# flanglet/kanzi

Hardware: AMD Instinct MI355X
Metric: encode+decode MB/s, 4 MiB-block synthetic stream, BWT+RANK+ZRLT & ANS0 (level-5 core chain), bit-exact .knz (higher is better)
Workload: dtype u8; 1 GPU; configs[2]: BWT+RANK+ZRLT & ANS0, 2048 x 4194304 B blocks per GPU per step (64 distinct synthetic blocks per GPU, SURVEY 8d generator standing in for silesia.tar, tiled), blocks round-robin over ranks; block_size=4194304, parallelism=blocks%1, round_trip_ok=True

## Files before the change

kanzi_amd/csrc/kz_ans.hip:

```cpp
#include "kz_device.h"
#include "kz_internal.h"
#include "kz_chunk.h"

typedef uint16_t u16;

#define ANS_TOP (1u << 15)
#define ANS_LR 12


struct BitW { u8* p; u32 pos; };
__device__ __forceinline__ void bw_put(BitW& w, u32 v, int count) {
  while (count > 0) {
    const int bitoff = w.pos & 7, room = 8 - bitoff;
    const int take = count < room ? count : room;
    const u32 bits = (v >> (count - take)) & ((1u << take) - 1u);
    w.p[w.pos >> 3] |= (u8)(bits << (room - take));
    w.pos += take; count -= take;
  }
}

typedef u16 __attribute__((aligned(1))) ans_u16_unaligned;
typedef u64 __attribute__((aligned(1))) ans_u64_unaligned;

__global__ __launch_bounds__(64) void k_ans_enc_chunk(const u8* __restrict__ src, int64_t stride,
                                                       const int32_t* __restrict__ d_len, AnsEnc E) {
  const int b = blockIdx.y, ck = blockIdx.x;
  const int count = d_len[b];
  const int lane = kz_lane();
  const int64_t ci = (int64_t)b * E.C + ck;
  const u8* blk = src + (int64_t)b * stride;
  u8* hdr = E.hdr + ci * ANS_HDR_BYTES;
  u8* scr = E.scr + ci * ANS_SCRATCH;
  if (count <= 32) {
    if (ck != 0) return;
    if (lane < count) scr[lane] = blk[lane];
    if (lane == 0) { E.hdrBits[ci] = 0; E.tailOff[ci] = 0; E.tailBits[ci] = 8u * (u32)count; }
    return;
  }
  const int start = ck * ANS_CHUNK;
  if (start >= count) return;
  const int end = min(count, start + ANS_CHUNK);
  const int len = end - start;

  __shared__ u32 hist[256];
  __shared__ u16 nfreq[256];
  __shared__ u8 alpha[256];
  __shared__ uint4 symTab[256];
  const u8* data = blk + start;
  __shared__ u32 hbuf[ANS_HDR_BYTES / 4];

  for (int i = lane; i < 256; i += 64) hist[i] = 0;
  for (int i = lane; i < ANS_HDR_BYTES / 4; i += 64) hbuf[i] = 0;
  __syncthreads();
  for (int i = lane * 4; i < len; i += 256) {
    u32 w = 0; int nb = min(4, len - i);
    if (nb == 4 && ((start + i) & 3) == 0) w = *(const u32*)(blk + start + i);
    else for (int k = 0; k < nb; k++) w |= (u32)blk[start + i + k] << (8 * k);
    for (int k = 0; k < 4; k++) {
      const bool valid = k < nb;
      const u32 c = (w >> (8 * k)) & 0xFF;
      const uint64_t peers = kz_match8(c, valid);
      if (valid && (peers & kz_lanemask_lt()) == 0) atomicAdd(&hist[c], (u32)__popcll(peers));
    }
  }
  __syncthreads();

  const u32 total = (u32)len, scale = 1u << ANS_LR;
  u32 f[4]; bool present[4];
  u32 alphabetSize = 0;
  u32 apos[4];
#pragma unroll
  for (int q = 0; q < 4; q++) {
    f[q] = hist[q * 64 + lane];
// ... 58 lines not shown
          if (adjustments == 0) break;
        }
#pragma unroll
        for (int q = 0; q < 4; q++) if (q == mq && lane == ml) { int v = (int)f[q] - delta; f[q] = (u32)(v > 1 ? v : 1); }
      }
      if (adjMax != 0) {
#pragma unroll
        for (int q = 0; q < 4; q++) if (q == mq && lane == ml) f[q] = (u32)((int)f[q] + adjMax);
      }
    }
  }
  u32 cum = 0;
#pragma unroll
  for (int q = 0; q < 4; q++) {
    const u32 fv = present[q] ? f[q] : 0;
    const u32 inc = kz_wave_incl_sum(fv);
    const u32 cumFreq = cum + inc - fv;
    cum += __shfl(inc, 63, 64);
    const int s = q * 64 + lane;
    nfreq[s] = (u16)fv;
    if (present[q]) {
      u32 freq = fv;
      if (freq >= scale) freq = scale - 1;
      const u32 xmaxv = ((ANS_TOP >> ANS_LR) << 16) * freq;
      const u32 cmplv = scale - freq;
      if (freq < 2) symTab[s] = make_uint4(xmaxv, 0xFFFFFFFFu, cumFreq + scale - 1, cmplv | (32u << 16));
      else {
        int shift = 0;
        while (freq > (1u << shift)) shift++;
        symTab[s] = make_uint4(xmaxv, (u32)((((1ULL << (shift + 31)) + freq - 1) / freq) & 0xFFFFFFFFULL), cumFreq, cmplv | ((u32)(32 + shift - 1) << 16));
      }
    }
  }
  __syncthreads();
  u32 hb = 0;
  if (lane == 0) {
    BitW w{(u8*)hbuf, 0};
    bw_put(w, ANS_LR - 8, 3);
    if (alphabetSize == 256) { bw_put(w, 0, 1); bw_put(w, 0, 1); }
    else if (alphabetSize == 0) { bw_put(w, 0, 1); bw_put(w, 1, 1); }
    else {
      bw_put(w, 1, 1);
      const int lastMask = alpha[alphabetSize - 1] >> 3;
      bw_put(w, (u32)lastMask, 5);
      for (int i = 0; i <= lastMask; i++) {
        u32 m = 0;
        for (int j = 0; j < 8; j++) if (nfreq[i * 8 + j] != 0) m |= 1u << j;
        bw_put(w, m, 8);
      }
    }
    if (alphabetSize > 1) {
      const int chkSize = (alphabetSize >= 64) ? 8 : 6;
      int llr = 3;
      while ((1 << llr) <= ANS_LR) llr++;
      for (int i = 1; i < (int)alphabetSize; i += chkSize) {
        const int endj = (i + chkSize < (int)alphabetSize) ? i + chkSize : (int)alphabetSize;
        int mx = (int)nfreq[alpha[i]] - 1;
        for (int j = i + 1; j < endj; j++) { int v = (int)nfreq[alpha[j]] - 1; if (v > mx) mx = v; }
        int logMax = 0;
        while ((1 << logMax) <= mx) logMax++;
        bw_put(w, (u32)logMax, llr);
        if (logMax == 0) continue;
        for (int j = i; j < endj; j++) bw_put(w, (u32)nfreq[alpha[j]] - 1u, logMax);
      }
    }
    hb = w.pos;
    E.hdrBits[ci] = hb;
  }
  __syncthreads();
  for (int i = lane; i < ANS_HDR_BYTES / 4; i += 64) ((u32*)hdr)[i] = hbuf[i];
  if (alphabetSize <= 1) {
    if (lane == 0) { E.tailOff[ci] = 0; E.tailBits[ci] = 0; }
    return;
  }
  const int bufLen = ANS_SCRATCH;
  const int end4 = len & -4;
  int n = bufLen - 1;
  if (lane == 0) for (int i = len - 1; i >= end4; i--) scr[n - (len - 1 - i)] = data[i];
  n -= (len - end4);
  u32 st = ANS_TOP;
  int idx = n;
  if (lane < 4) {
#define ANS_ENC_STEP(WD)                                                                                      \
    { const u32 c = ((WD) >> (8 * (3 - lane))) & 0xFFu;                                                       \
      const uint4 sy = symTab[c];                                                                             \
      const bool x = st >= sy.x;                                               \
      const uint64_t bal = kz_ballot(x) & 0xFULL;                                                             \
      const int pre = (int)__popcll(bal & kz_lanemask_lt());                                                  \
      if (x) {                                                       \
        const int e = idx - 2 * pre;                                                                          \
        *(ans_u16_unaligned*)(scr + e - 1) = (u16)(((st & 0xFFu) << 8) | ((st >> 8) & 0xFFu));                \
        st >>= 16;                                                                                            \
      }                                                                                                       \
      idx -= 2 * (int)__popcll(bal);                                                                          \
      const u32 q = (u32)(((u64)st * (u64)sy.y) >> (sy.w >> 16));                                             \
      st = st + sy.z + q * (sy.w & 0xFFFFu); }
    const int T = end4 >> 2;
    const uint4* d16 = (const uint4*)data;
    int g = (T - 1) >> 2;
    uint4 cur = (T > 0) ? d16[g] : make_uint4(0, 0, 0, 0);
    for (; g >= 0; g--) {
      const uint4 nxt = (g > 0) ? d16[g - 1] : make_uint4(0, 0, 0, 0);
      const int top = min(3, T - 1 - 4 * g);
      if (top >= 3) ANS_ENC_STEP(cur.w)
      if (top >= 2) ANS_ENC_STEP(cur.z)
      if (top >= 1) ANS_ENC_STEP(cur.y)
      ANS_ENC_STEP(cur.x)
      cur = nxt;
    }
#undef ANS_ENC_STEP
  }
  idx = __shfl(idx, 0, 64);
  n = idx + 1;
  const u32 payload = (u32)(bufLen - n);
  u32 vlen = 1; { u32 v = payload; while (v >= 128) { v >>= 7; vlen++; } }
  const int tail = n - 16 - (int)vlen;
  if (lane == 0) {
    u32 v = payload; int p = tail;
    while (v >= 128) { scr[p++] = (u8)(0x80 | (v & 0x7F)); v >>= 7; }
    scr[p++] = (u8)v;
    E.tailOff[ci] = (u32)tail; E.tailBits[ci] = 8u * (payload + 16 + vlen);
  }
  if (lane < 4) {
    u8* p = scr + tail + vlen + 4 * lane;
    p[0] = (u8)(st >> 24); p[1] = (u8)(st >> 16); p[2] = (u8)(st >> 8); p[3] = (u8)st;
  }
}

__global__ __launch_bounds__(64) void k_ans_enc_scan(const int32_t* __restrict__ d_len, AnsEnc E, int64_t* __restrict__ d_bits, int rawLimit) {
  const int b = blockIdx.x;
  const int count = d_len[b];
  const int chunks = (count <= rawLimit) ? (count > 0 ? 1 : 0) : (count + E.chunk - 1) / E.chunk;
  const int lane = kz_lane();
  u64 carry = 0;
  for (int base = 0; base < chunks; base += 64) {
    const int c = base + lane;
    const int64_t ci = (int64_t)b * E.C + c;
    const u32 v = (c < chunks) ? E.hdrBits[ci] + E.tailBits[ci] : 0;
    const u32 inc = kz_wave_incl_sum(v);
    if (c < chunks) E.bitOff[ci] = carry + inc - v;
    carry += __shfl(inc, 63, 64);
  }
  if (lane == 0) d_bits[b] = (int64_t)carry;
}

__device__ __forceinline__ u32 kz_fetch32(const u8* __restrict__ p, int64_t nbits, int64_t r) {
  if (r >= nbits || r + 32 <= 0) return 0;
  u64 acc = 0;
  const int64_t byte0 = (r >= 0) ? (r >> 3) : -((-r + 7) >> 3);
// ... 52 lines not shown
  E.hdrBits = (u32*)kz_arena_alloc(ctx, (size_t)B * E.C * 4);
  E.tailOff = (u32*)kz_arena_alloc(ctx, (size_t)B * E.C * 4);
  E.tailBits = (u32*)kz_arena_alloc(ctx, (size_t)B * E.C * 4);
  E.bitOff = (u64*)kz_arena_alloc(ctx, (size_t)B * E.C * 8);
  if (!E.bitOff || !E.scr) { snprintf(ctx->err, sizeof(ctx->err), "entropy encode: arena overflow"); return -KZ_ERR_DEVICE; }
  KZ_HIP(hipMemsetAsync(E.hdrBits, 0, (size_t)B * E.C * 4, ctx->stream));
  KZ_HIP(hipMemsetAsync(E.tailBits, 0, (size_t)B * E.C * 4, ctx->stream));
  *chunksOut = (maxN + ANS_CHUNK - 1) / ANS_CHUNK;
  return 0;
}
int kz_chunk_enc_finish(kz_ctx* ctx, kz_batch& bt, AnsEnc& E, int chunks, uint8_t* out, int64_t outStride,
                        const int32_t* d_hdrBytes, int64_t* d_bits, int rawLimit) {
  const int B = bt.B;
  KZ_LAUNCH(ctx, KID_ANS_ENC_SCAN, k_ans_enc_scan, dim3(B), dim3(64), bt.d_len, E, d_bits, rawLimit);
  if (chunks > 0) KZ_LAUNCH(ctx, KID_ANS_ENC_CONCAT, k_ans_enc_concat, dim3(chunks, B), dim3(KZ_WG), bt.d_len, E, out, outStride, d_hdrBytes, rawLimit);
  KZ_HIP(hipGetLastError());
  return 0;
}

int kz_stage_ans0_encode(kz_ctx* ctx, kz_batch& bt, uint8_t* out, int64_t outStride, const int32_t* d_hdrBytes, int64_t* d_bits) {
  AnsEnc E; int chunks = 0;
  int rc = kz_chunk_enc_alloc(ctx, bt, E, &chunks);
  if (rc) return rc;
  if (chunks > 0) KZ_LAUNCH(ctx, KID_ANS_ENC_CHUNK, k_ans_enc_chunk, dim3(chunks, bt.B), dim3(64), bt.buf[bt.cur], bt.stride, bt.d_len, E);
  return kz_chunk_enc_finish(ctx, bt, E, chunks, out, outStride, d_hdrBytes, d_bits, 32);
}

#define ANS_EV_NONE 0x7FFFFFFF
#define ANS_EV_FAIL 0
#define ANS_EV_SKIP 1
#define ANS_EV_STOP 2
#define ANS_MAX_CHUNK_SIZE (1u << 27)
struct AnsDec {
  u64* chunkBit;
  int32_t* event;
  int32_t* nIdx;
  int32_t* hdrOnly;
  int C;
};

__device__ __forceinline__ u32 kz_peek(const u8* __restrict__ p, u64 pos, int count) {
  const u64 by = pos >> 3;
  u32 acc = ((u32)p[by] << 24) | ((u32)p[by + 1] << 16) | ((u32)p[by + 2] << 8) | (u32)p[by + 3];
  acc <<= (pos & 7);
  return count ? (acc >> (32 - count)) : 0;
}

// ... 53 lines not shown
  D.event[b] = event;
  D.nIdx[b] = nIdx;
  D.hdrOnly[b] = hdrOnly;
}

__device__ __forceinline__ void ans_fill_f2s(const u16* __restrict__ cumf, u8* __restrict__ f2s, int scale, int lane) {
  const int x0 = lane * 64;
  if (x0 >= scale) return;
  int lo = 0, hi = 256;
  while (hi - lo > 1) { const int mid = (lo + hi) >> 1; if ((int)cumf[mid] <= x0) lo = mid; else hi = mid; }
  int sy = lo;
  int nextAt = (sy + 1 < 256) ? (int)cumf[sy + 1] : 0x7FFFFFFF;
  for (int x = x0; x < x0 + 64; x += 4) {
    u32 w = 0;
#pragma unroll
    for (int k = 0; k < 4; k++) {
      while (nextAt <= x + k) { sy++; nextAt = (sy + 1 < 256) ? (int)cumf[sy + 1] : 0x7FFFFFFF; }
      w |= (u32)sy << (8 * k);
    }
    *(u32*)(f2s + x) = w;
  }
}

__global__ __launch_bounds__(64) void k_ans_dec_chunk(const u8* __restrict__ in, int64_t inStride, const int64_t* __restrict__ d_bitOff,
                                                       const int32_t* __restrict__ d_len, AnsDec D, u8* __restrict__ dst, int64_t stride) {
  const int b = blockIdx.y, ck = blockIdx.x;
  const int count = d_len[b];
  const int lane = kz_lane();
  const u8* p = in + (int64_t)b * inStride;
  u8* o = dst + (int64_t)b * stride;
  if (count <= 32) {
    if (ck != 0) return;
    if (lane < count) o[lane] = (u8)kz_peek(p, (u64)d_bitOff[b] + 8ULL * lane, 8);
    return;
  }
  const int start = ck * ANS_CHUNK;
  if (start >= count || ck >= D.nIdx[b]) return;
  const int end = min(count, start + ANS_CHUNK);
  __shared__ u16 freq[256];
  __shared__ u16 cumf[256];
  __shared__ u8 alpha[256];
  __shared__ __attribute__((aligned(4))) u8 f2s[4096];
  __shared__ int sh_asz, sh_lr, sh_bad;
  __shared__ u64 sh_pos;
  for (int i = lane; i < 256; i += 64) freq[i] = 0;
  __syncthreads();
  if (lane == 0) {
    u64 pos = D.chunkBit[(int64_t)b * D.C + ck];
    int bad = 0;
    const int lr = 8 + (int)kz_peek(p, pos, 3); pos += 3;
    const int scale = 1 << lr;
    int asz = 0;
    if (kz_peek(p, pos, 1) == 0) {
      if (kz_peek(p, pos + 1, 1) == 1) asz = 0; else { asz = 256; for (int i = 0; i < 256; i++) alpha[i] = (u8)i; }
      pos += 2;
    } else {
      const int lastMask = (int)kz_peek(p, pos + 1, 5); pos += 6;
      for (int i = 0; i <= lastMask; i++) {
        const u32 m = kz_peek(p, pos, 8); pos += 8;
        for (int j = 0; j < 8; j++) if (m & (1u << j)) alpha[asz++] = (u8)((i << 3) + j);
      }
    }
    if (asz > 0) {
      int llr = 3;
      while ((1 << llr) <= lr) llr++;
      const int chkSize = (asz >= 64) ? 8 : 6;
      int sum = 0;
      for (int i = 1; i < asz && !bad; i += chkSize) {
        const int logMax = (int)kz_peek(p, pos, llr); pos += llr;
        if ((1 << logMax) > scale) { bad = 1; break; }
        const int endj = (i + chkSize < asz) ? i + chkSize : asz;
        for (int j = i; j < endj; j++) {
          const int fq = (logMax == 0) ? 1 : 1 + (int)kz_peek(p, pos, logMax);
          pos += logMax;
          if (fq <= 0 || fq >= scale) { bad = 1; break; }
          freq[alpha[j]] = (u16)fq; sum += fq;
        }
      }
      if (scale <= sum) bad = 1;
      if (!bad) freq[alpha[0]] = (u16)(scale - sum);
    }
    sh_asz = asz; sh_lr = lr; sh_bad = bad; sh_pos = pos;
  }
  __syncthreads();
  const int asz = sh_asz, lr = sh_lr;
  if (sh_bad || asz == 0) { if (lane == 0) atomicMin(&D.event[b], ck * 4 + ANS_EV_FAIL); return; }
  if (ck == D.hdrOnly[b]) return;
  if (asz == 1) {
    const u8 c = alpha[0];
    for (int i = start + lane; i < end; i += 64) o[i] = c;
    return;
  }
  u32 cum = 0;
#pragma unroll
  for (int q = 0; q < 4; q++) {
    const u32 fv = freq[q * 64 + lane];
    const u32 inc = kz_wave_incl_sum(fv);
    cumf[q * 64 + lane] = (u16)(cum + inc - fv);
    cum += __shfl(inc, 63, 64);
  }
  __syncthreads();
  const bool wide = lr > 12;
  if (!wide) ans_fill_f2s(cumf, f2s, 1 << lr, lane);
  __syncthreads();
  u64 pos = sh_pos;
  u32 v = kz_peek(p, pos, 8); pos += 8;
  u32 sz = v & 0x7F; int shift = 7;
  while (v >= 128) { v = kz_peek(p, pos, 8); pos += 8; sz |= (v & 0x7F) << shift; if (shift == 28) break; shift += 7; }
  u32 st = 0;
  if (lane < 4) { const u64 sp = pos + 32ULL * (3 - lane); st = (kz_peek(p, sp, 16) << 16) | kz_peek(p, sp + 16, 16); }
  pos += 128;
  const u64 payloadBit = pos;
  const u32 mask = (1u << lr) - 1u;
  const int len = end - start;
  const int end4 = len & -4;
  u32 n = 0;
  if (lane < 4) {
    const u64 payByte = payloadBit >> 3;
    const u32 payShift = (u32)(payloadBit & 7);
    const bool winOk = payByte + (u64)sz + 48 <= (u64)inStride;
    u32 wbase = 0;
    u64 rHi = 0, rLo = 0, rNx = 0, rNx2 = 0;
    if (winOk) {
      rHi = __builtin_bswap64(*(const ans_u64_unaligned*)(p + payByte));
      rLo = __builtin_bswap64(*(const ans_u64_unaligned*)(p + payByte + 8));
      rNx = *(const ans_u64_unaligned*)(p + payByte + 16);
      rNx2 = *(const ans_u64_unaligned*)(p + payByte + 24);
    }
    for (int i = 0; i < end4; i += 4) {
      if (winOk && n > wbase + 7) {
        rHi = rLo; rLo = __builtin_bswap64(rNx); rNx = rNx2; wbase += 8;
        rNx2 = *(const ans_u64_unaligned*)(p + payByte + min(wbase, sz) + 24);
      }
      u32 cur;
      if (!wide) cur = f2s[st & mask];
      else {
        const u32 x = st & mask;
        int lo = 0, hi = 256;
        while (hi - lo > 1) { const int mid = (lo + hi) >> 1; if ((u32)cumf[mid] <= x) lo = mid; else hi = mid; }
        cur = (u32)lo;
      }
      o[start + i + lane] = (u8)cur;
      u32 fq = freq[cur]; if (fq >= (1u << lr)) fq = (1u << lr) - 1u;
      st = fq * (st >> lr) + (st & mask) - (u32)cumf[cur];
      const bool need = (int)st < (int)ANS_TOP;
      const uint64_t bal = kz_ballot(need) & 0xFULL;
      if (need) {
        const u32 off = 2u * (u32)__popcll(bal & kz_lanemask_lt());
        const u32 at = n + off;
        u32 hi, lo;
        if (winOk) {
          const u32 bp = 8u * (at - wbase) + payShift;
          const u64 v = (bp < 64) ? ((rHi << bp) | (bp ? (rLo >> (64 - bp)) : 0ULL)) : (rLo << (bp - 64));
          const u32 two = (u32)(v >> 48);
          hi = (at < sz) ? (two >> 8) : 0u; lo = (at + 1 < sz) ? (two & 0xFFu) : 0u;
        }
        else { hi = (at < sz) ? kz_peek(p, payloadBit + 8ULL * at, 8) : 0; lo = (at + 1 < sz) ? kz_peek(p, payloadBit + 8ULL * (at + 1), 8) : 0; }
        st = (st << 16) | (hi << 8) | lo;
      }
      n += 2u * (u32)__popcll(bal);
    }
  }
  n = __shfl(n, 0, 64);
  if (lane < len - end4) { const u32 at = n + (u32)lane; o[start + end4 + lane] = (at < sz) ? (u8)kz_peek(p, payloadBit + 8ULL * at, 8) : 0; }
  n += (u32)(len - end4);
  if (lane == 0 && n != sz) atomicMin(&D.event[b], ck * 4 + ANS_EV_STOP);
}

__global__ __launch_bounds__(64) void k_ans_dec_fin(const int32_t* __restrict__ d_len, int32_t* __restrict__ d_len2, int32_t* __restrict__ d_flag,
                                                     AnsDec D, u8* __restrict__ dst, int64_t stride, long long* __restrict__ endOut) {
  const int b = blockIdx.x, lane = kz_lane();
  const int count = d_len[b];
  const int ev = D.event[b];
  if (lane == 0) { d_len2[b] = count; d_flag[b] = (ev == ANS_EV_NONE || (ev & 3) != ANS_EV_FAIL) ? 1 : 0; }
  if (ev == ANS_EV_NONE || (ev & 3) == ANS_EV_FAIL) return;
  if (endOut && lane == 0 && (ev & 3) == ANS_EV_STOP) endOut[b] = (long long)D.chunkBit[(int64_t)b * D.C + (ev >> 2) + 1];
  const int64_t from = (int64_t)((ev >> 2) + ((ev & 3) == ANS_EV_STOP ? 1 : 0)) * ANS_CHUNK;
  u8* o = dst + (int64_t)b * stride;
  for (int64_t i = from + lane; i < count; i += 64) o[i] = 0;
}

int kz_stage_ans0_decode(kz_ctx* ctx, kz_batch& bt, const uint8_t* in, int64_t inStride, const int64_t* d_bitOff, const int64_t* d_bitEnd) {
  const int B = bt.B;
  int maxN = 0;
  for (int b = 0; b < B; b++) if (bt.h_len[b] > maxN) maxN = bt.h_len[b];
  AnsDec D;
  D.C = (maxN + ANS_CHUNK - 1) / ANS_CHUNK + 1;
  D.chunkBit = (u64*)kz_arena_alloc(ctx, (size_t)B * D.C * 8);
  D.event = (int32_t*)kz_arena_alloc(ctx, (size_t)B * 4);
  D.nIdx = (int32_t*)kz_arena_alloc(ctx, (size_t)B * 4);
  D.hdrOnly = (int32_t*)kz_arena_alloc(ctx, (size_t)B * 4);
  if (!D.event || !D.nIdx || !D.hdrOnly || !D.chunkBit) { snprintf(ctx->err, sizeof(ctx->err), "ans0_decode: arena overflow"); return -KZ_ERR_DEVICE; }
  hipStream_t st = ctx->stream;
  u8* dst = bt.buf[bt.cur ^ 1];
  KZ_LAUNCH(ctx, KID_ANS_DEC_INDEX, k_ans_dec_index, dim3((B + 63) / 64), dim3(64), in, inStride, d_bitOff, d_bitEnd, bt.d_len, D, B, ctx->d_endBits);
  const int chunks = (maxN + ANS_CHUNK - 1) / ANS_CHUNK;
  if (chunks > 0) KZ_LAUNCH(ctx, KID_ANS_DEC_CHUNK, k_ans_dec_chunk, dim3(chunks, B), dim3(64), in, inStride, d_bitOff, bt.d_len, D, dst, bt.stride);
  KZ_LAUNCH(ctx, KID_ANS_DEC_FIN, k_ans_dec_fin, dim3(B), dim3(64), bt.d_len, bt.d_len2, bt.d_flag, D, dst, bt.stride, ctx->d_endBits);
  KZ_HIP(hipGetLastError());
  bt.cur ^= 1;
  { int32_t* t = bt.d_len; bt.d_len = bt.d_len2; bt.d_len2 = t; }
  return 0;
}
```

kanzi_amd/csrc/kz_api.hip:

```cpp
#include <dirent.h>
#include "kz_pipe.h"
#include <stdlib.h>
#include <thread>
#include <sched.h>

extern "C" int32_t kz_abi_version(void) { return KZ_ABI_VERSION; }

extern "C" kz_ctx* kz_ctx_create(int32_t deviceId) {
  int ndev = 0;
  if (hipGetDeviceCount(&ndev) != hipSuccess || ndev <= 0) return nullptr;
  if (deviceId < 0 || deviceId >= ndev) return nullptr;
  if (hipSetDevice(deviceId) != hipSuccess) return nullptr;
  kz_ctx* ctx = new kz_ctx();
  ctx->device = deviceId;
  { int cus = 0; if (hipDeviceGetAttribute(&cus, hipDeviceAttributeMultiprocessorCount, deviceId) == hipSuccess && cus > 0) ctx->numCUs = cus; }
  if (hipStreamCreateWithFlags(&ctx->stream, hipStreamNonBlocking) != hipSuccess) { delete ctx; return nullptr; }
  if (hipHostMalloc((void**)&ctx->hpin, 1 << 20, hipHostMallocDefault) != hipSuccess) { hipStreamDestroy(ctx->stream); delete ctx; return nullptr; }
  ctx->hpinInts = (1 << 20) / 4;
  kz_switches_read(ctx->sw);
  {
    const int hw = (int)std::thread::hardware_concurrency();
    ctx->blockingWaits = ctx->sw.blockingWaits >= 0 ? ctx->sw.blockingWaits : ((hw > 0 && kz_usable_cpus() < hw) ? 1 : 0);
  }
  return ctx;
// ... 13 lines not shown
  s.utfGpu = digit("KZ_UTF_GPU", 0, 0, 1);
  s.utfFwdGpu = digit("KZ_UTF_FWD_GPU", 0, 1, -1);
  s.textGpuTrace = flag("KZ_TEXT_GPU_TRACE");
  s.fuseMinBlocks = num("KZ_FUSE_MIN_BLOCKS", 32);
  s.overlapClasses = num("KZ_OVERLAP_CLASSES", 3);
  { const char* e = getenv("KZ_WIDE_QUEUES"); s.wideQueues = e ? (atoi(e) ? 1 : 0) : -1; }
  s.noSFirst = flag("KZ_NO_SFIRST");
  s.traceSched = flag("KZ_TRACE_SCHED");
  s.tracePipe = flag("KZ_TRACE_PIPE");
  s.hostChunk = num("KZ_HOST_CHUNK", 0);
  { const int v = num("KZ_HOST_CHUNK_DEC", 512); s.hostChunkDec = v < 8 ? 8 : v; }
  { const char* e = getenv("KZ_HOST_INV_STAGED"); s.hostInvStaged = e ? atoi(e) : -1; }
  s.streamChunk = num("KZ_STREAM_CHUNK", 0);
  s.streamSerial = flag("KZ_STREAM_SERIAL");
  s.readScatter = flag("KZ_READ_SCATTER");
  s.writeGather = flag("KZ_WRITE_GATHER");
  s.bwtTrie = num("KZ_BWT_TRIE", -1); s.bwtTrieWin = num("KZ_BWT_TRIEWIN", -1); s.bwtBuckets = num("KZ_BWT_BUCKETS", -1);
  s.bwtDmax = num("KZ_BWT_DMAX", -1); s.bwtRetire = num("KZ_BWT_RETIRE", -1); s.bwtLazyRank = num("KZ_BWT_LAZYRANK", -1);
  s.bwtTrace = flag("KZ_BWT_TRACE");
  s.bwtTestTrieOverflow = digit("KZ_BWT_TEST_TRIE_OVERFLOW", 0, 9, -1);
  s.cmTestRowBytes = num("KZ_CM_TEST_ROW_BYTES", 0);
  { const char* f = getenv("KZ_FPAQ_FORCE"); s.fpaqForce = f ? ((f[0] == 'w' || f[0] == 'W' || f[0] == '1') ? 1 : ((f[0] == 'l' || f[0] == 'L' || f[0] == '2') ? 2 : 0)) : 0; }
  s.sbrtForm = num("KZ_SBRT_FORM", -1);
}
extern "C" void kz_ctx_reload_switches(kz_ctx* ctx) {
  if (!ctx) return;
  kz_switches_read(ctx->sw);
  if (ctx->sw.blockingWaits >= 0) ctx->blockingWaits = ctx->sw.blockingWaits;
}
extern "C" void kz_ctx_destroy(kz_ctx* ctx) {
  if (!ctx) return;
  if (ctx->worker.joinable()) {
    { std::lock_guard<std::mutex> g(ctx->qmu); ctx->stopWorker = true; }
    ctx->qcv.notify_all();
    ctx->worker.join();
  }
  hipSetDevice(ctx->device);
  if (ctx->arena) hipFree(ctx->arena);
  for (int i = 0; i < 5; i++) { if (ctx->side[i]) hipStreamDestroy(ctx->side[i]); if (ctx->evJoin[i]) hipEventDestroy(ctx->evJoin[i]); }
  if (ctx->hpin) hipHostFree(ctx->hpin);
  for (int i = 0; i < 2; i++) {
    if (ctx->pinIn[i].p) hipHostFree(ctx->pinIn[i].p);
    if (ctx->pinOut[i].p) hipHostFree(ctx->pinOut[i].p);
    if (ctx->hsIn[i].p) hipHostFree(ctx->hsIn[i].p);
    if (ctx->hsOut[i].p) hipHostFree(ctx->hsOut[i].p);
    if (ctx->tfOut[i].p) hipHostFree(ctx->tfOut[i].p);
// ... 362 lines not shown
```

kanzi_amd/csrc/kz_internal.h:

```cpp
#pragma once
#include <hip/hip_runtime.h>
#include <stdint.h>
#include <stdio.h>
#include <string.h>
#include <vector>
#include <condition_variable>
#include <deque>
#include <functional>
#include <map>
#include <set>
#include <mutex>
#include <thread>
#include "../../include/kanzi_hip.h"

#define KZ_KERNELS(X) \
  X(KID_ANS_ENC_CHUNK, "k_ans_enc_chunk") X(KID_ANS_ENC_SCAN, "k_ans_enc_scan") X(KID_ANS_ENC_CONCAT, "k_ans_enc_concat") X(KID_ANS_DEC_INDEX, "k_ans_dec_index") \
  X(KID_ANS_DEC_CHUNK, "k_ans_dec_chunk") X(KID_ANS_DEC_FIN, "k_ans_dec_fin") X(KID_MASK_LEN, "k_mask_len") X(KID_PASSTHROUGH, "k_passthrough") \
  X(KID_FRAME_PREPARE, "k_frame_prepare") X(KID_COPY_BYTES, "k_copy_bytes") X(KID_FRAME_DECIDE, "k_frame_decide") X(KID_FRAME_HEADER, "k_frame_header") \
  X(KID_FRAME_PARSE, "k_frame_parse") X(KID_COPY_PAYLOAD, "k_copy_payload") X(KID_BWT_INIT, "k_bwt_init") X(KID_RADIX_HIST, "k_radix_hist") \
  X(KID_RADIX_SCAN, "k_radix_scan") X(KID_RADIX_SCATTER, "k_radix_scatter") X(KID_SEG_REDUCE, "k_seg_reduce") X(KID_SEG_SCAN, "k_seg_scan") \
  X(KID_SEG_APPLY, "k_seg_apply") X(KID_LIVE_EMIT, "k_live_emit") X(KID_BWT_EMIT, "k_bwt_emit") X(KID_BWTI_PARSE, "k_bwti_parse") \
  X(KID_BWTI_HIST, "k_bwti_hist") X(KID_BWTI_SCAN, "k_bwti_scan") X(KID_BWTI_SCATTER, "k_bwti_scatter") X(KID_BWTI_WALK1, "k_bwti_walk1") \
  X(KID_BWTI_RESOLVE, "k_bwti_resolve") X(KID_BWTI_COPY, "k_bwti_copy") X(KID_BWTI_LITERAL, "k_bwti_literal") X(KID_BWTI_FIN, "k_bwti_fin") \
  X(KID_SBRT_LAST2, "k_sbrt_last2") X(KID_SBRT_SCAN, "k_sbrt_scan") X(KID_SBRT_REPLAY, "k_sbrt_replay") X(KID_COPY_LEN, "k_copy_len") \
// ... 39 lines not shown
  int utfGpu = 1;
  int utfFwdGpu = -1;
  int textGpuTrace = 0;
  int fuseMinBlocks = 32;
  int overlapClasses = 3;
  int wideQueues = -1;
  int noSFirst = 0;
  int traceSched = 0;
  int tracePipe = 0;
  int hostChunk = 0;
  int hostChunkDec = 512;
  int hostInvStaged = -1;
  int streamChunk = 0;
  int streamSerial = 0;
  int readScatter = 0;
  int writeGather = 0;
  int bwtTrie = -1, bwtTrieWin = -1, bwtBuckets = -1, bwtDmax = -1, bwtRetire = -1;
  int bwtLazyRank = -1;
  int bwtTrace = 0;
  int bwtTestTrieOverflow = -1;
  int fpaqForce = 0;
  int cmTestRowBytes = 0;
  int sbrtForm = -1;
};
void kz_switches_read(kz_switches& s);

struct KzPending { hipEvent_t e0, e1; int id; };
struct kz_ctx {
  int device = 0;
  kz_switches sw;
  hipStream_t stream = nullptr;
  hipStream_t side[5] = {nullptr, nullptr, nullptr, nullptr, nullptr};
  hipEvent_t evJoin[5] = {nullptr, nullptr, nullptr, nullptr, nullptr};
  int wideQueues = -1;
  int wideNow = 0;
  uint8_t* arena = nullptr;
  size_t arenaCap = 0, arenaTop = 0;
  int32_t* hpin = nullptr;
  size_t hpinInts = 0;
  char err[512] = {0};
  float stageMs[KZ_MAX_STAGES] = {0};
  int64_t stageAlgBytes[KZ_MAX_STAGES] = {0};
  int nStages = 0;
  int checksum = 0;
  int skipBlocks = 0;
  int dataType = 0;
// ... 205 lines not shown
```

Baseline: 5046 MB/s.

## Pack multiple ANS chunks per wavefront in encode and decode kernels

The ANS encode and decode kernels previously ran one chunk per 64-lane wave, with only 4 lanes active in the serial coding loop. They now process N chunks (default 4) per workgroup, giving each chunk a 4-lane group, so more lanes do useful work and fewer workgroups are launched. Other changes ride along: a compact 8-byte symbol table, deferred stores in the encoder, and a shared-memory byte-swapped ring buffer for decoder refill bytes. The cost is more shared memory per workgroup, serialized per-chunk setup, and idle lanes when chunks differ in length.

```diff
diff --git a/kanzi_amd/csrc/kz_ans.hip b/kanzi_amd/csrc/kz_ans.hip
--- a/kanzi_amd/csrc/kz_ans.hip
+++ b/kanzi_amd/csrc/kz_ans.hip
@@ -6,6 +6,9 @@
 
 #define ANS_TOP (1u << 15)
 #define ANS_LR 12
+#define ANS_PACK_ENC 4
+#define ANS_PACK_DEC 4
+static int kz_ans_pack(int sw, int dflt) { return (sw == 1 || sw == 4 || sw == 8 || sw == 16) ? sw : dflt; }
 
 
 struct BitW { u8* p; u32 pos; };
@@ -21,34 +24,12 @@
 
 typedef u16 __attribute__((aligned(1))) ans_u16_unaligned;
 typedef u64 __attribute__((aligned(1))) ans_u64_unaligned;
-
-__global__ __launch_bounds__(64) void k_ans_enc_chunk(const u8* __restrict__ src, int64_t stride,
-                                                       const int32_t* __restrict__ d_len, AnsEnc E) {
-  const int b = blockIdx.y, ck = blockIdx.x;
-  const int count = d_len[b];
-  const int lane = kz_lane();
-  const int64_t ci = (int64_t)b * E.C + ck;
-  const u8* blk = src + (int64_t)b * stride;
+typedef u64 __attribute__((may_alias)) ans_u64_alias;
+typedef u16 __attribute__((may_alias)) ans_u16_alias;
+
+__device__ __forceinline__ bool ans_enc_prepare(const u8* __restrict__ blk, int start, int len, int64_t ci, const AnsEnc& E, u32* hist, u16* nfreq,
+                                                u8* alpha, u32* hbuf, uint2* symTab, int lane) {
   u8* hdr = E.hdr + ci * ANS_HDR_BYTES;
-  u8* scr = E.scr + ci * ANS_SCRATCH;
-  if (count <= 32) {
-    if (ck != 0) return;
-    if (lane < count) scr[lane] = blk[lane];
-    if (lane == 0) { E.hdrBits[ci] = 0; E.tailOff[ci] = 0; E.tailBits[ci] = 8u * (u32)count; }
-    return;
-  }
-  const int start = ck * ANS_CHUNK;
-  if (start >= count) return;
-  const int end = min(count, start + ANS_CHUNK);
-  const int len = end - start;
-
-  __shared__ u32 hist[256];
-  __shared__ u16 nfreq[256];
-  __shared__ u8 alpha[256];
-  __shared__ uint4 symTab[256];
-  const u8* data = blk + start;
-  __shared__ u32 hbuf[ANS_HDR_BYTES / 4];
-
   for (int i = lane; i < 256; i += 64) hist[i] = 0;
   for (int i = lane; i < ANS_HDR_BYTES / 4; i += 64) hbuf[i] = 0;
   __syncthreads();
@@ -153,13 +134,11 @@
     if (present[q]) {
       u32 freq = fv;
       if (freq >= scale) freq = scale - 1;
-      const u32 xmaxv = ((ANS_TOP >> ANS_LR) << 16) * freq;
-      const u32 cmplv = scale - freq;
-      if (freq < 2) symTab[s] = make_uint4(xmaxv, 0xFFFFFFFFu, cumFreq + scale - 1, cmplv | (32u << 16));
+      if (freq < 2) symTab[s] = make_uint2(0xFFFFFFFFu, freq | ((cumFreq + scale - 1) << 12));
       else {
         int shift = 0;
         while (freq > (1u << shift)) shift++;
-        symTab[s] = make_uint4(xmaxv, (u32)((((1ULL << (shift + 31)) + freq - 1) / freq) & 0xFFFFFFFFULL), cumFreq, cmplv | ((u32)(32 + shift - 1) << 16));
+        symTab[s] = make_uint2((u32)((((1ULL << (shift + 31)) + freq - 1) / freq) & 0xFFFFFFFFULL), freq | (cumFreq << 12) | ((u32)(shift - 1) << 25));
       }
     }
   }
@@ -202,60 +181,112 @@
   for (int i = lane; i < ANS_HDR_BYTES / 4; i += 64) ((u32*)hdr)[i] = hbuf[i];
   if (alphabetSize <= 1) {
     if (lane == 0) { E.tailOff[ci] = 0; E.tailBits[ci] = 0; }
+    return false;
+  }
+  return true;
+}
+__device__ __forceinline__ u32 ans_group4(bool p, int gsh) {
+  return (u32)(__builtin_amdgcn_ballot_w64(p) >> gsh) & 0xFu;
+}
+
+template <int N>
+__global__ __launch_bounds__(64) void k_ans_enc_chunk(const u8* __restrict__ src, int64_t stride,
+                                                       const int32_t* __restrict__ d_len, AnsEnc E) {
+  const int b = blockIdx.y, ck0 = blockIdx.x * N;
+  const int count = d_len[b];
+  const int lane = kz_lane();
+  const u8* blk = src + (int64_t)b * stride;
+  if (count <= 32) {
+    if (ck0 != 0) return;
+    const int64_t ci = (int64_t)b * E.C;
+    u8* scr = E.scr + ci * ANS_SCRATCH;
+    if (lane < count) scr[lane] = blk[lane];
+    if (lane == 0) { E.hdrBits[ci] = 0; E.tailOff[ci] = 0; E.tailBits[ci] = 8u * (u32)count; }
     return;
   }
+  if (ck0 * ANS_CHUNK >= count) return;
+
+  __shared__ u32 hist[256];
+  __shared__ u16 nfreq[256];
+  __shared__ u8 alpha[256];
+  __shared__ u32 hbuf[ANS_HDR_BYTES / 4];
+  __shared__ uint2 symTab[N][256];
+  __shared__ int codeLen[N];
+  for (int j = 0; j < N; j++) {
+    const int start = (ck0 + j) * ANS_CHUNK;
+    int len = 0;
+    if (start < count) {
+      len = min(count - start, ANS_CHUNK);
+      if (!ans_enc_prepare(blk, start, len, (int64_t)b * E.C + ck0 + j, E, hist, nfreq, alpha, hbuf, symTab[j], lane)) len = 0;
+    }
+    if (lane == 0) codeLen[j] = len;
+    __syncthreads();
+  }
+  const int j = lane >> 2, sub = lane & 3, gsh = lane & 60;
+  const int len = (j < N) ? codeLen[j < N ? j : 0] : 0;
+  const bool act = len > 0;
+  const int64_t ci = (int64_t)b * E.C + ck0 + (act ? j : 0);
+  const u8* data = blk + (int64_t)(ck0 + (act ? j : 0)) * ANS_CHUNK;
+  u8* scr = E.scr + ci * ANS_SCRATCH;
+  const uint2* tab = symTab[j < N ? j : 0];
   const int bufLen = ANS_SCRATCH;
   const int end4 = len & -4;
-  int n = bufLen - 1;
-  if (lane == 0) for (int i = len - 1; i >= end4; i--) scr[n - (len - 1 - i)] = data[i];
-  n -= (len - end4);
+  if (act && sub == 0) for (int i = len - 1; i >= end4; i--) scr[bufLen - 1 - (len - 1 - i)] = data[i];
+  int idx = bufLen - 1 - (len - end4);
   u32 st = ANS_TOP;
-  int idx = n;
-  if (lane < 4) {
-#define ANS_ENC_STEP(WD)                                                                                      \
-    { const u32 c = ((WD) >> (8 * (3 - lane))) & 0xFFu;                                                       \
-      const uint4 sy = symTab[c];                                                                             \
-      const bool x = st >= sy.x;                                               \
-      const uint64_t bal = kz_ballot(x) & 0xFULL;                                                             \
-      const int pre = (int)__popcll(bal & kz_lanemask_lt());                                                  \
-      if (x) {                                                       \
-        const int e = idx - 2 * pre;                                                                          \
-        *(ans_u16_unaligned*)(scr + e - 1) = (u16)(((st & 0xFFu) << 8) | ((st >> 8) & 0xFFu));                \
-        st >>= 16;                                                                                            \
-      }                                                                                                       \
-      idx -= 2 * (int)__popcll(bal);                                                                          \
-      const u32 q = (u32)(((u64)st * (u64)sy.y) >> (sy.w >> 16));                                             \
-      st = st + sy.z + q * (sy.w & 0xFFFFu); }
-    const int T = end4 >> 2;
-    const uint4* d16 = (const uint4*)data;
-    int g = (T - 1) >> 2;
-    uint4 cur = (T > 0) ? d16[g] : make_uint4(0, 0, 0, 0);
-    for (; g >= 0; g--) {
-      const uint4 nxt = (g > 0) ? d16[g - 1] : make_uint4(0, 0, 0, 0);
-      const int top = min(3, T - 1 - 4 * g);
-      if (top >= 3) ANS_ENC_STEP(cur.w)
-      if (top >= 2) ANS_ENC_STEP(cur.z)
-      if (top >= 1) ANS_ENC_STEP(cur.y)
-      ANS_ENC_STEP(cur.x)
-      cur = nxt;
-    }
+#define ANS_ENC_STEP(WD, ON, PK)                                                                              \
+  { const u32 c = ((WD) >> (8 * (3 - sub))) & 0xFFu;                                                          \
+    const uint2 sy = tab[c];                                                                                  \
+    const u32 fq = sy.y & 0xFFFu;                                                                             \
+    const bool x = (ON) && st >= (fq << 19);                            \
+    const u32 grp = ans_group4(x, gsh);                                                      \
+    const u32 e1 = (u32)(idx - 1 - 2 * (int)__popc(grp & ((1u << sub) - 1u)));                                \
+    PK = x ? ((e1 << 16) | ((st & 0xFFu) << 8) | ((st >> 8) & 0xFFu)) : 0u;                                   \
+    if (x) st >>= 16;                                                                                         \
+    idx -= 2 * (int)__popc(grp);                                                                              \
+    if (ON) {                                                                                                 \
+      const u32 q = __umulhi(st, sy.x) >> (sy.y >> 25);              \
+      st = st + ((sy.y >> 12) & 0x1FFFu) + q * ((1u << ANS_LR) - fq); } }
+#define ANS_ENC_PUT(PK) if (PK) *(ans_u16_unaligned*)(scr + ((PK) >> 16)) = (u16)(PK);
+  const int T = end4 >> 2;
+  const int G = act ? (T - 1) >> 2 : -1;
+  int Gmax = G;
+#pragma unroll
+  for (int d = 32; d > 0; d >>= 1) Gmax = max(Gmax, __shfl_xor(Gmax, d, 64));
+  const uint4* d16 = (const uint4*)data;
+  uint4 cur0 = d16[max(min(Gmax, G), 0)], cur1 = d16[max(min(Gmax - 1, G), 0)];
+  for (int g = Gmax; g >= 0; g -= 2) {
+    const bool in0 = g <= G, in1 = g - 1 <= G && g >= 1;
+    const uint4 nxt0 = d16[max(min(g - 2, G), 0)], nxt1 = d16[max(min(g - 3, G), 0)];
+    const int top0 = T - 1 - 4 * g, top1 = top0 + 4;
+    u32 pk0, pk1, pk2, pk3, pk4, pk5, pk6, pk7;
+    ANS_ENC_STEP(cur0.w, in0 && top0 >= 3, pk0)
+    ANS_ENC_STEP(cur0.z, in0 && top0 >= 2, pk1)
+    ANS_ENC_STEP(cur0.y, in0 && top0 >= 1, pk2)
+    ANS_ENC_STEP(cur0.x, in0, pk3)
+    ANS_ENC_STEP(cur1.w, in1 && top1 >= 3, pk4)
+    ANS_ENC_STEP(cur1.z, in1 && top1 >= 2, pk5)
+    ANS_ENC_STEP(cur1.y, in1 && top1 >= 1, pk6)
+    ANS_ENC_STEP(cur1.x, in1, pk7)
+    cur0 = nxt0; cur1 = nxt1;
+    asm volatile("" : "+v"(cur0.x), "+v"(cur0.y), "+v"(cur0.z), "+v"(cur0.w), "+v"(cur1.x), "+v"(cur1.y), "+v"(cur1.z), "+v"(cur1.w) : : "memory");
+    ANS_ENC_PUT(pk0) ANS_ENC_PUT(pk1) ANS_ENC_PUT(pk2) ANS_ENC_PUT(pk3) ANS_ENC_PUT(pk4) ANS_ENC_PUT(pk5) ANS_ENC_PUT(pk6) ANS_ENC_PUT(pk7)
+  }
 #undef ANS_ENC_STEP
-  }
-  idx = __shfl(idx, 0, 64);
-  n = idx + 1;
+#undef ANS_ENC_PUT
+  if (!act) return;
+  const int n = idx + 1;
   const u32 payload = (u32)(bufLen - n);
   u32 vlen = 1; { u32 v = payload; while (v >= 128) { v >>= 7; vlen++; } }
   const int tail = n - 16 - (int)vlen;
-  if (lane == 0) {
+  if (sub == 0) {
     u32 v = payload; int p = tail;
     while (v >= 128) { scr[p++] = (u8)(0x80 | (v & 0x7F)); v >>= 7; }
     scr[p++] = (u8)v;
     E.tailOff[ci] = (u32)tail; E.tailBits[ci] = 8u * (payload + 16 + vlen);
   }
-  if (lane < 4) {
-    u8* p = scr + tail + vlen + 4 * lane;
-    p[0] = (u8)(st >> 24); p[1] = (u8)(st >> 16); p[2] = (u8)(st >> 8); p[3] = (u8)st;
-  }
+  u8* p = scr + tail + vlen + 4 * sub;
+  p[0] = (u8)(st >> 24); p[1] = (u8)(st >> 16); p[2] = (u8)(st >> 8); p[3] = (u8)st;
 }
 
 __global__ __launch_bounds__(64) void k_ans_enc_scan(const int32_t* __restrict__ d_len, AnsEnc E, int64_t* __restrict__ d_bits, int rawLimit) {
@@ -354,7 +385,16 @@
   AnsEnc E; int chunks = 0;
   int rc = kz_chunk_enc_alloc(ctx, bt, E, &chunks);
   if (rc) return rc;
-  if (chunks > 0) KZ_LAUNCH(ctx, KID_ANS_ENC_CHUNK, k_ans_enc_chunk, dim3(chunks, bt.B), dim3(64), bt.buf[bt.cur], bt.stride, bt.d_len, E);
+  if (chunks > 0) {
+#define ANS_ENC_LAUNCH(N) KZ_LAUNCH(ctx, KID_ANS_ENC_CHUNK, k_ans_enc_chunk<N>, dim3((chunks + N - 1) / N, bt.B), dim3(64), bt.buf[bt.cur], bt.stride, bt.d_len, E)
+    switch (kz_ans_pack(ctx->sw.ansPackEnc, ANS_PACK_ENC)) {
+      case 1: ANS_ENC_LAUNCH(1); break;
+      case 4: ANS_ENC_LAUNCH(4); break;
+      case 8: ANS_ENC_LAUNCH(8); break;
+      default: ANS_ENC_LAUNCH(16); break;
+    }
+#undef ANS_ENC_LAUNCH
+  }
   return kz_chunk_enc_finish(ctx, bt, E, chunks, out, outStride, d_hdrBytes, d_bits, 32);
 }
 
@@ -454,31 +494,37 @@
   }
 }
 
+#define ANS_RING 256
+#define ANS_RING_Q 64
+#define ANS_RING_K 8
+template <int N>
 __global__ __launch_bounds__(64) void k_ans_dec_chunk(const u8* __restrict__ in, int64_t inStride, const int64_t* __restrict__ d_bitOff,
                                                        const int32_t* __restrict__ d_len, AnsDec D, u8* __restrict__ dst, int64_t stride) {
-  const int b = blockIdx.y, ck = blockIdx.x;
+  const int b = blockIdx.y, ck0 = blockIdx.x * N;
   const int count = d_len[b];
   const int lane = kz_lane();
   const u8* p = in + (int64_t)b * inStride;
   u8* o = dst + (int64_t)b * stride;
   if (count <= 32) {
-    if (ck != 0) return;
+    if (ck0 != 0) return;
     if (lane < count) o[lane] = (u8)kz_peek(p, (u64)d_bitOff[b] + 8ULL * lane, 8);
     return;
   }
-  const int start = ck * ANS_CHUNK;
-  if (start >= count || ck >= D.nIdx[b]) return;
-  const int end = min(count, start + ANS_CHUNK);
-  __shared__ u16 freq[256];
-  __shared__ u16 cumf[256];
-  __shared__ u8 alpha[256];
-  __shared__ __attribute__((aligned(4))) u8 f2s[4096];
-  __shared__ int sh_asz, sh_lr, sh_bad;
-  __shared__ u64 sh_pos;
-  for (int i = lane; i < 256; i += 64) freq[i] = 0;
+  const int nch = min(N, min(D.nIdx[b], (count + ANS_CHUNK - 1) / ANS_CHUNK) - ck0);
+  if (nch <= 0) return;
+  __shared__ u16 freq[N][256];
+  __shared__ u16 cumf[N][256];
+  __shared__ __attribute__((aligned(8))) u8 f2s[N][4096];
+  __shared__ __attribute__((aligned(8))) u8 ring[N][ANS_RING];
+  __shared__ int sh_asz[N], sh_lr[N], sh_bad[N], sh_act[N];
+  __shared__ u64 sh_pos[N];
+  for (int i = lane; i < N * 256; i += 64) (&freq[0][0])[i] = 0;
+  if (lane < N) sh_act[lane] = 0;
   __syncthreads();
-  if (lane == 0) {
-    u64 pos = D.chunkBit[(int64_t)b * D.C + ck];
+  if (lane < nch) {
+    u16* fr = freq[lane];
+    u8* alpha = f2s[lane];
+    u64 pos = D.chunkBit[(int64_t)b * D.C + ck0 + lane];
     int bad = 0;
     const int lr = 8 + (int)kz_peek(p, pos, 3); pos += 3;
     const int scale = 1 << lr;
@@ -490,7 +536,7 @@
       const int lastMask = (int)kz_peek(p, pos + 1, 5); pos += 6;
       for (int i = 0; i <= lastMask; i++) {
         const u32 m = kz_peek(p, pos, 8); pos += 8;
-        for (int j = 0; j < 8; j++) if (m & (1u << j)) alpha[asz++] = (u8)((i << 3) + j);
+        for (int k = 0; k < 8; k++) if (m & (1u << k)) alpha[asz++] = (u8)((i << 3) + k);
       }
     }
     if (asz > 0) {
@@ -502,101 +548,132 @@
         const int logMax = (int)kz_peek(p, pos, llr); pos += llr;
         if ((1 << logMax) > scale) { bad = 1; break; }
         const int endj = (i + chkSize < asz) ? i + chkSize : asz;
-        for (int j = i; j < endj; j++) {
+        for (int k = i; k < endj; k++) {
           const int fq = (logMax == 0) ? 1 : 1 + (int)kz_peek(p, pos, logMax);
           pos += logMax;
           if (fq <= 0 || fq >= scale) { bad = 1; break; }
-          freq[alpha[j]] = (u16)fq; sum += fq;
+          fr[alpha[k]] = (u16)fq; sum += fq;
         }
       }
       if (scale <= sum) bad = 1;
-      if (!bad) freq[alpha[0]] = (u16)(scale - sum);
-    }
-    sh_asz = asz; sh_lr = lr; sh_bad = bad; sh_pos = pos;
+      if (!bad) fr[alpha[0]] = (u16)(scale - sum);
+    }
+    sh_asz[lane] = asz; sh_lr[lane] = lr; sh_bad[lane] = bad; sh_pos[lane] = pos;
   }
   __syncthreads();
-  const int asz = sh_asz, lr = sh_lr;
-  if (sh_bad || asz == 0) { if (lane == 0) atomicMin(&D.event[b], ck * 4 + ANS_EV_FAIL); return; }
-  if (ck == D.hdrOnly[b]) return;
-  if (asz == 1) {
-    const u8 c = alpha[0];
-    for (int i = start + lane; i < end; i += 64) o[i] = c;
-    return;
-  }
-  u32 cum = 0;
-#pragma unroll
-  for (int q = 0; q < 4; q++) {
-    const u32 fv = freq[q * 64 + lane];
-    const u32 inc = kz_wave_incl_sum(fv);
-    cumf[q * 64 + lane] = (u16)(cum + inc - fv);
-    cum += __shfl(inc, 63, 64);
+  const int hdrOnly = D.hdrOnly[b];
+  for (int c = 0; c < nch; c++) {
+    const int ck = ck0 + c, start = ck * ANS_CHUNK, end = min(count, start + ANS_CHUNK);
+    const int asz = sh_asz[c], lr = sh_lr[c];
+    if (sh_bad[c] || asz == 0) { if (lane == 0) atomicMin(&D.event[b], ck * 4 + ANS_EV_FAIL); continue; }
+    if (ck == hdrOnly) continue;
+    if (asz == 1) {
+      const u8 sym = f2s[c][0];
+      for (int i = start + lane; i < end; i += 64) o[i] = sym;
+      continue;
+    }
+    u32 cum = 0;
+#pragma unroll
+    for (int q = 0; q < 4; q++) {
+      const u32 fv = freq[c][q * 64 + lane];
+      const u32 inc = kz_wave_incl_sum(fv);
+      cumf[c][q * 64 + lane] = (u16)(cum + inc - fv);
+      cum += __shfl(inc, 63, 64);
+    }
+    __syncthreads();
+    if (lr <= 12) ans_fill_f2s(cumf[c], f2s[c], 1 << lr, lane);
+    if (lane == 0) sh_act[c] = 1;
   }
   __syncthreads();
+  const int j = (lane >> 2) < N ? (lane >> 2) : 0, sub = lane & 3, gsh = lane & 60;
+  const bool act = (lane >> 2) < N && sh_act[j] != 0;
+  const int ck = ck0 + j, start = ck * ANS_CHUNK;
+  const int len = act ? min(count - start, ANS_CHUNK) : 0;
+  const int end4 = len & -4;
+  const int lr = act ? sh_lr[j] : 12;
+  const u32 mask = (1u << lr) - 1u;
   const bool wide = lr > 12;
-  if (!wide) ans_fill_f2s(cumf, f2s, 1 << lr, lane);
-  __syncthreads();
-  u64 pos = sh_pos;
-  u32 v = kz_peek(p, pos, 8); pos += 8;
-  u32 sz = v & 0x7F; int shift = 7;
-  while (v >= 128) { v = kz_peek(p, pos, 8); pos += 8; sz |= (v & 0x7F) << shift; if (shift == 28) break; shift += 7; }
-  u32 st = 0;
-  if (lane < 4) { const u64 sp = pos + 32ULL * (3 - lane); st = (kz_peek(p, sp, 16) << 16) | kz_peek(p, sp + 16, 16); }
+  const u16* fr = freq[j];
+  const u16* cf = cumf[j];
+  const u8* f2 = f2s[j];
+  u8* rg = ring[j];
+  u64 pos = act ? sh_pos[j] : 0;
+  u32 sz = 0, st = 0;
+  if (act) {
+    u32 v = kz_peek(p, pos, 8); pos += 8;
+    sz = v & 0x7F; int shift = 7;
+    while (v >= 128) { v = kz_peek(p, pos, 8); pos += 8; sz |= (v & 0x7F) << shift; if (shift == 28) break; shift += 7; }
+    const u64 sp = pos + 32ULL * (3 - sub);
+    st = (kz_peek(p, sp, 16) << 16) | kz_peek(p, sp + 16, 16);
+  }
   pos += 128;
   const u64 payloadBit = pos;
-  const u32 mask = (1u << lr) - 1u;
-  const int len = end - start;
-  const int end4 = len & -4;
+  const u64 payByte = payloadBit >> 3;
+  const u32 payShift = (u32)(payloadBit & 7);
+  const bool winOk = act && payByte + (u64)sz + 48 <= (u64)inStride;
+  u64 r0, r1, r2;
+#define ANS_RING_LOAD(OFF) { const u8* a_ = p + (winOk ? payByte + (u64)min((u32)(OFF), sz) : 0ULL);                            \
+    r0 = *(const ans_u64_unaligned*)a_; r1 = *(const ans_u64_unaligned*)(a_ + 8); r2 = *(const ans_u64_unaligned*)(a_ + 16); }
+#define ANS_RING_PUT(OFF) { const u64 b0_ = __builtin_bswap64(r0), b1_ = __builtin_bswap64(r1), b2_ = __builtin_bswap64(r2);     \
+    ans_u64_alias* q_ = (ans_u64_alias*)(rg + ((u32)(OFF) & (ANS_RING - 1)));                                                                         \
+    q_[0] = payShift ? ((b0_ << payShift) | (b1_ >> (64 - payShift))) : b0_;                                                      \
+    q_[1] = payShift ? ((b1_ << payShift) | (b2_ >> (64 - payShift))) : b1_; }
+  u32 filled = 0;
+  for (; filled < 2 * ANS_RING_Q; filled += ANS_RING_Q) {
+    ANS_RING_LOAD(filled + 16 * sub)
+    if (winOk) ANS_RING_PUT(filled + 16 * sub)
+  }
+  ANS_RING_LOAD(filled + 16 * sub)
+  bool pend = winOk;
+  int maxEnd4 = end4;
+#pragma unroll
+  for (int d = 32; d > 0; d >>= 1) maxEnd4 = max(maxEnd4, __shfl_xor(maxEnd4, d, 64));
   u32 n = 0;
-  if (lane < 4) {
-    const u64 payByte = payloadBit >> 3;
-    const u32 payShift = (u32)(payloadBit & 7);
-    const bool winOk = payByte + (u64)sz + 48 <= (u64)inStride;
-    u32 wbase = 0;
-    u64 rHi = 0, rLo = 0, rNx = 0, rNx2 = 0;
-    if (winOk) {
-      rHi = __builtin_bswap64(*(const ans_u64_unaligned*)(p + payByte));
-      rLo = __builtin_bswap64(*(const ans_u64_unaligned*)(p + payByte + 8));
-      rNx = *(const ans_u64_unaligned*)(p + payByte + 16);
-      rNx2 = *(const ans_u64_unaligned*)(p + payByte + 24);
-    }
-    for (int i = 0; i < end4; i += 4) {
-      if (winOk && n > wbase + 7) {
-        rHi = rLo; rLo = __builtin_bswap64(rNx); rNx = rNx2; wbase += 8;
-        rNx2 = *(const ans_u64_unaligned*)(p + payByte + min(wbase, sz) + 24);
-      }
-      u32 cur;
-      if (!wide) cur = f2s[st & mask];
-      else {
-        const u32 x = st & mask;
-        int lo = 0, hi = 256;
-        while (hi - lo > 1) { const int mid = (lo + hi) >> 1; if ((u32)cumf[mid] <= x) lo = mid; else hi = mid; }
-        cur = (u32)lo;
-      }
-      o[start + i + lane] = (u8)cur;
-      u32 fq = freq[cur]; if (fq >= (1u << lr)) fq = (1u << lr) - 1u;
-      st = fq * (st >> lr) + (st & mask) - (u32)cumf[cur];
-      const bool need = (int)st < (int)ANS_TOP;
-      const uint64_t bal = kz_ballot(need) & 0xFULL;
-      if (need) {
-        const u32 off = 2u * (u32)__popcll(bal & kz_lanemask_lt());
-        const u32 at = n + off;
-        u32 hi, lo;
-        if (winOk) {
-          const u32 bp = 8u * (at - wbase) + payShift;
-          const u64 v = (bp < 64) ? ((rHi << bp) | (bp ? (rLo >> (64 - bp)) : 0ULL)) : (rLo << (bp - 64));
-          const u32 two = (u32)(v >> 48);
-          hi = (at < sz) ? (two >> 8) : 0u; lo = (at + 1 < sz) ? (two & 0xFFu) : 0u;
+  for (int i0 = 0; i0 < maxEnd4; i0 += 4 * ANS_RING_K) {
+    u32 out0 = 0, out1 = 0;
+#pragma unroll
+    for (int k = 0; k < ANS_RING_K; k++) {
+      const int i = i0 + 4 * k;
+      if (i < end4) {
+        u32 cur;
+        if (!wide) cur = f2[st & mask];
+        else {
+          const u32 x = st & mask;
+          int lo = 0, hi = 256;
+          while (hi - lo > 1) { const int mid = (lo + hi) >> 1; if ((u32)cf[mid] <= x) lo = mid; else hi = mid; }
+          cur = (u32)lo;
         }
-        else { hi = (at < sz) ? kz_peek(p, payloadBit + 8ULL * at, 8) : 0; lo = (at + 1 < sz) ? kz_peek(p, payloadBit + 8ULL * (at + 1), 8) : 0; }
-        st = (st << 16) | (hi << 8) | lo;
-      }
-      n += 2u * (u32)__popcll(bal);
-    }
-  }
-  n = __shfl(n, 0, 64);
-  if (lane < len - end4) { const u32 at = n + (u32)lane; o[start + end4 + lane] = (at < sz) ? (u8)kz_peek(p, payloadBit + 8ULL * at, 8) : 0; }
+        if (k < 4) out0 |= cur << (8 * k); else out1 |= cur << (8 * (k - 4));
+        u32 fq = fr[cur]; if (fq >= (1u << lr)) fq = (1u << lr) - 1u;
+        st = fq * (st >> lr) + (st & mask) - (u32)cf[cur];
+        const bool need = (int)st < (int)ANS_TOP;
+        const u32 grp = ans_group4(need, gsh);
+        if (need) {
+          const u32 at = n + 2u * (u32)__popc(grp & ((1u << sub) - 1u));
+          u32 hi, lo;
+          if (winOk) {
+            const u32 two = *(const ans_u16_alias*)(rg + ((at & (ANS_RING - 1)) ^ 6u));
+            hi = (at < sz) ? (two >> 8) : 0u; lo = (at + 1 < sz) ? (two & 0xFFu) : 0u;
+          }
+          else { hi = (at < sz) ? kz_peek(p, payloadBit + 8ULL * at, 8) : 0; lo = (at + 1 < sz) ? kz_peek(p, payloadBit + 8ULL * (at + 1), 8) : 0; }
+          st = (st << 16) | (hi << 8) | lo;
+        }
+        n += 2u * (u32)__popc(grp);
+      }
+    }
+    if (pend) { ANS_RING_PUT(filled + 16 * sub) filled += ANS_RING_Q; }
+#pragma unroll
+    for (int k = 0; k < ANS_RING_K; k++)
+      if (i0 + 4 * k < end4) o[start + i0 + 4 * k + sub] = (u8)((k < 4 ? out0 : out1) >> (8 * (k & 3)));
+    pend = winOk && filled - n <= ANS_RING - ANS_RING_Q;
+    ANS_RING_LOAD(filled + 16 * sub)
+  }
+#undef ANS_RING_LOAD
+#undef ANS_RING_PUT
+  if (!act) return;
+  if (sub < len - end4) { const u32 at = n + (u32)sub; o[start + end4 + sub] = (at < sz) ? (u8)kz_peek(p, payloadBit + 8ULL * at, 8) : 0; }
   n += (u32)(len - end4);
-  if (lane == 0 && n != sz) atomicMin(&D.event[b], ck * 4 + ANS_EV_STOP);
+  if (sub == 0 && n != sz) atomicMin(&D.event[b], ck * 4 + ANS_EV_STOP);
 }
 
 __global__ __launch_bounds__(64) void k_ans_dec_fin(const int32_t* __restrict__ d_len, int32_t* __restrict__ d_len2, int32_t* __restrict__ d_flag,
@@ -627,7 +704,16 @@
   u8* dst = bt.buf[bt.cur ^ 1];
   KZ_LAUNCH(ctx, KID_ANS_DEC_INDEX, k_ans_dec_index, dim3((B + 63) / 64), dim3(64), in, inStride, d_bitOff, d_bitEnd, bt.d_len, D, B, ctx->d_endBits);
   const int chunks = (maxN + ANS_CHUNK - 1) / ANS_CHUNK;
-  if (chunks > 0) KZ_LAUNCH(ctx, KID_ANS_DEC_CHUNK, k_ans_dec_chunk, dim3(chunks, B), dim3(64), in, inStride, d_bitOff, bt.d_len, D, dst, bt.stride);
+  if (chunks > 0) {
+#define ANS_DEC_LAUNCH(N) KZ_LAUNCH(ctx, KID_ANS_DEC_CHUNK, k_ans_dec_chunk<N>, dim3((chunks + N - 1) / N, B), dim3(64), in, inStride, d_bitOff, bt.d_len, D, dst, bt.stride)
+    switch (kz_ans_pack(ctx->sw.ansPackDec, ANS_PACK_DEC)) {
+      case 1: ANS_DEC_LAUNCH(1); break;
+      case 4: ANS_DEC_LAUNCH(4); break;
+      case 8: ANS_DEC_LAUNCH(8); break;
+      default: ANS_DEC_LAUNCH(16); break;
+    }
+#undef ANS_DEC_LAUNCH
+  }
   KZ_LAUNCH(ctx, KID_ANS_DEC_FIN, k_ans_dec_fin, dim3(B), dim3(64), bt.d_len, bt.d_len2, bt.d_flag, D, dst, bt.stride, ctx->d_endBits);
   KZ_HIP(hipGetLastError());
   bt.cur ^= 1;
diff --git a/kanzi_amd/csrc/kz_api.hip b/kanzi_amd/csrc/kz_api.hip
--- a/kanzi_amd/csrc/kz_api.hip
+++ b/kanzi_amd/csrc/kz_api.hip
@@ -59,6 +59,8 @@
   s.cmTestRowBytes = num("KZ_CM_TEST_ROW_BYTES", 0);
   { const char* f = getenv("KZ_FPAQ_FORCE"); s.fpaqForce = f ? ((f[0] == 'w' || f[0] == 'W' || f[0] == '1') ? 1 : ((f[0] == 'l' || f[0] == 'L' || f[0] == '2') ? 2 : 0)) : 0; }
   s.sbrtForm = num("KZ_SBRT_FORM", -1);
+  s.ansPackEnc = num("KZ_ANS_PACK_ENC", num("KZ_ANS_PACK", 0));
+  s.ansPackDec = num("KZ_ANS_PACK_DEC", num("KZ_ANS_PACK", 0));
 }
 extern "C" void kz_ctx_reload_switches(kz_ctx* ctx) {
   if (!ctx) return;
diff --git a/kanzi_amd/csrc/kz_internal.h b/kanzi_amd/csrc/kz_internal.h
--- a/kanzi_amd/csrc/kz_internal.h
+++ b/kanzi_amd/csrc/kz_internal.h
@@ -85,6 +85,7 @@
   int fpaqForce = 0;
   int cmTestRowBytes = 0;
   int sbrtForm = -1;
+  int ansPackEnc = 0, ansPackDec = 0;
 };
 void kz_switches_read(kz_switches& s);
 
```

Result: no change. 5086 MB/s, median of 6 (+0.8%).
